# shizhenneko/Video-Transformer

Hardware: AMD Instinct MI355X
Metric: 720p frames/sec decoded+scored per node; segment-index exact-match vs CPU (higher is better)
Workload: dtype u8; 1 GPU; decode_score: BASELINE config [3] per-GPU share: 4 x 10-min 720p MP4 per GPU (config [3] = 32 videos over 8 GPUs; at N GPUs 4N videos, video i on rank i mod N) through vtseg.batch.plan_batch; synthetic H.264 1280x720 @30fps, 4 x 18000 frames (10.0 min) per GPU, thumbnails k=4; config_name=720p-batch, videos=4, videos_per_gpu=4, frames_per_video=18000, frames_per_gpu=72000, width=1280, height=720, k=4, parallelism=video-per-gpu x1 (video i on rank i mod 1), hw_queues=4, recon_launches=120, windows=1

## Files before the change

### video-transformer_amd/csrc/decode.hip

```cpp
#include <hip/hip_runtime.h>

#include <cstdint>

#include "common.h"
#include "decode.h"
#include "h264.h"
#include "parse_slice.h"
#include "pixel.h"

namespace vts {
namespace {

#ifndef VTS_PARSE_WAVES
#define VTS_PARSE_WAVES 0
#endif
#if VTS_PARSE_WAVES
#define VTS_PARSE_OCC __attribute__((amdgpu_waves_per_eu(VTS_PARSE_WAVES)))
#else
#define VTS_PARSE_OCC
#endif
__global__ void __launch_bounds__(64) VTS_PARSE_OCC h264_parse(ParseArgs a) {
  __shared__ ParseScratch scratch[64];
  const int s = blockIdx.x * blockDim.x + threadIdx.x;
  if (s >= a.n_slices) return;
  const SliceDesc sd = a.slices[s];
  const uint32_t errs = parse_slice(a.es, sd.nal_offset, sd.nal_size, sd.slot, sd.ref_slot, a.prm, a.cmd,
                                    &scratch[threadIdx.x], a.epoch);
  if (errs) atomicOr(a.err, errs);
}

__device__ __forceinline__ uint4 load16_any(const uint8_t *p) {
  const int sh = static_cast<int>(reinterpret_cast<uintptr_t>(p) & 15);
  const uint4 *q = reinterpret_cast<const uint4 *>(p - sh);
  const uint4 lo = q[0];
  if (sh == 0) return lo;
  const uint4 hi = q[1];
  const uint32_t w[8] = {lo.x, lo.y, lo.z, lo.w, hi.x, hi.y, hi.z, hi.w};
  const int qd = sh >> 2, r = sh & 3;
  uint32_t s[5];
#pragma unroll
  for (int i = 0; i < 5; ++i)
    s[i] = (qd == 0) ? w[i] : (qd == 1) ? w[i + 1] : (qd == 2) ? w[i + 2] : w[i + 3 < 8 ? i + 3 : 7];
  return make_uint4(__builtin_amdgcn_alignbyte(s[1], s[0], r), __builtin_amdgcn_alignbyte(s[2], s[1], r),
                    __builtin_amdgcn_alignbyte(s[3], s[2], r), __builtin_amdgcn_alignbyte(s[4], s[3], r));
}

__device__ __forceinline__ uint32_t has_zero_byte(uint32_t v) {
  return (v - 0x01010101u) & ~v & 0x80808080u;
}

__device__ bool epb_in_pcm(const uint8_t *chunk, int n, const uint8_t *pcm) {
  for (int j = -2; j < n; ++j) {
    const uint8_t *t = chunk + j;
    if (t + 2 < pcm || t + 2 >= pcm + 384) continue;
    if (t[0] == 0 && t[1] == 0 && t[2] == 3) return true;
  }
  return false;
}

__device__ __noinline__ uint32_t pcm_rows_epb(const uint8_t *pcm, int q, int kk, int hk) {
  bool bad = false;
  for (int i = 0; i < kk; ++i) bad |= epb_in_pcm(pcm + 16 * (q * kk + i), 16, pcm);
  for (int i = 0; i < hk; ++i)
    bad |= epb_in_pcm(pcm + 256 + 8 * (q * hk + i), 8, pcm) || epb_in_pcm(pcm + 320 + 8 * (q * hk + i), 8, pcm);
  return bad ? DEC_E_EPB_IN_PCM : 0u;
}

__device__ __forceinline__ uint4 interleave_uv(uint32_t u0, uint32_t u1, uint32_t v0, uint32_t v1) {
  return make_uint4(__builtin_amdgcn_perm(v0, u0, 0x05010400u), __builtin_amdgcn_perm(v0, u0, 0x07030602u),
                    __builtin_amdgcn_perm(v1, u1, 0x05010400u), __builtin_amdgcn_perm(v1, u1, 0x07030602u));
}

__device__ __forceinline__ int clampi(int v, int lo, int hi) { return v < lo ? lo : (v > hi ? hi : v); }

constexpr int kReconThreads = 256;

#ifndef VTS_NT_LOAD
#define VTS_NT_LOAD 0
#endif
#ifndef VTS_NT_STORE
#define VTS_NT_STORE 1
#endif
typedef uint32_t u32x4 __attribute__((ext_vector_type(4)));

__device__ __forceinline__ uint4 ld_row(const uint4 *p) {
#if VTS_NT_LOAD
  const u32x4 v = __builtin_nontemporal_load(reinterpret_cast<const u32x4 *>(p));
  return make_uint4(v.x, v.y, v.z, v.w);
#else
  return *p;
#endif
}
__device__ __forceinline__ void st_row(uint8_t *p, const uint4 v) {
#if VTS_NT_STORE
  __builtin_nontemporal_store(u32x4{v.x, v.y, v.z, v.w}, reinterpret_cast<u32x4 *>(p));
#else
  *reinterpret_cast<uint4 *>(p) = v;
#endif
}

struct FrameRefs {
  const uint8_t *es;
  const uint8_t *ref, *ref_uv;
  int W, H, CW, CH;
  int64_t pitch;
};

__device__ __forceinline__ uint4 fetch_row(const FrameRefs &F, uint64_t c, int r, int m, int mby,
                                           uint32_t &errs) {
  const uint32_t kind = static_cast<uint32_t>(c >> 62);
  const int mvx = static_cast<int16_t>(c & 0xffff), mvy = static_cast<int16_t>((c >> 16) & 0xffff);
  uint4 out = make_uint4(0, 0, 0, 0);
  if (kind == 0 || (kind == 2 && !F.ref)) {
    errs |= (kind == 0) ? DEC_E_MISSING_MB : DEC_E_NO_REF;
  } else if (r < 16) {
    if (kind == 1) {
      const uint8_t *pcm = F.es + static_cast<int64_t>(c & 0xffffffffffffull);
      const uint8_t *src = pcm + 16 * r;
      out = load16_any(src);
      if ((has_zero_byte(out.x) | has_zero_byte(out.y) | has_zero_byte(out.z) | has_zero_byte(out.w)) &&
          epb_in_pcm(src, 16, pcm))
        errs |= DEC_E_EPB_IN_PCM;
    } else {
      const int sy = clampi(mby * 16 + r + (mvy >> 2), 0, F.H - 1);
      const int sx = m * 16 + (mvx >> 2);
      const uint8_t *row = F.ref + sy * F.pitch;
      if (sx >= 0 && sx + 15 <= F.W - 1) {
        out = load16_any(row + sx);
      } else {
        uint64_t lo8 = 0, hi8 = 0;
#pragma unroll 1
        for (int b = 0; b < 16; ++b) {
          const uint64_t v = row[clampi(sx + b, 0, F.W - 1)];
          if (b < 8) lo8 |= v << (8 * b); else hi8 |= v << (8 * (b - 8));
        }
        out = make_uint4(uint32_t(lo8), uint32_t(lo8 >> 32), uint32_t(hi8), uint32_t(hi8 >> 32));
      }
    }
  } else {
    const int cr = r - 16;
    if (kind == 1) {
      const uint8_t *pcm = F.es + static_cast<int64_t>(c & 0xffffffffffffull);
      const uint4 u = load16_any(pcm + 256 + 8 * cr);
      const uint4 v = load16_any(pcm + 320 + 8 * cr);
      out = interleave_uv(u.x, u.y, v.x, v.y);
      if ((has_zero_byte(u.x) | has_zero_byte(u.y) | has_zero_byte(v.x) | has_zero_byte(v.y)) &&
          (epb_in_pcm(pcm + 256 + 8 * cr, 8, pcm) || epb_in_pcm(pcm + 320 + 8 * cr, 8, pcm)))
        errs |= DEC_E_EPB_IN_PCM;
    } else {
      const int fx = mvx & 7, fy = mvy & 7;
      const int cx = m * 8 + (mvx >> 3), cy = mby * 8 + cr + (mvy >> 3);
      if (fx == 0 && fy == 0) {
        const uint8_t *row = F.ref_uv + clampi(cy, 0, F.CH - 1) * F.pitch;
        if (cx >= 0 && cx + 7 <= F.CW - 1) {
          out = load16_any(row + 2 * cx);
        } else {
          uint64_t lo8 = 0, hi8 = 0;
#pragma unroll 1
          for (int b = 0; b < 8; ++b) {
            const int sx = clampi(cx + b, 0, F.CW - 1);
            const uint64_t v = uint64_t(row[2 * sx]) | (uint64_t(row[2 * sx + 1]) << 8);
            if (b < 4) lo8 |= v << (16 * b); else hi8 |= v << (16 * (b - 4));
          }
          out = make_uint4(uint32_t(lo8), uint32_t(lo8 >> 32), uint32_t(hi8), uint32_t(hi8 >> 32));
        }
      } else {
        const uint8_t *ra = F.ref_uv + clampi(cy, 0, F.CH - 1) * F.pitch;
        const uint8_t *rb = F.ref_uv + clampi(cy + 1, 0, F.CH - 1) * F.pitch;
        uint64_t lo8 = 0, hi8 = 0;
#pragma unroll 1
        for (int b = 0; b < 8; ++b) {
          const int xa = clampi(cx + b, 0, F.CW - 1), xb = clampi(cx + b + 1, 0, F.CW - 1);
          uint64_t pair = 0;
#pragma unroll
          for (int pl = 0; pl < 2; ++pl) {
            const int A = ra[2 * xa + pl], B = ra[2 * xb + pl], C = rb[2 * xa + pl], D = rb[2 * xb + pl];
            const uint64_t v = static_cast<uint64_t>(
                ((8 - fx) * (8 - fy) * A + fx * (8 - fy) * B + (8 - fx) * fy * C + fx * fy * D + 32) >> 6);
            pair |= v << (8 * pl);
          }
          if (b < 4) lo8 |= pair << (16 * b); else hi8 |= pair << (16 * (b - 4));
        }
        out = make_uint4(uint32_t(lo8), uint32_t(lo8 >> 32), uint32_t(hi8), uint32_t(hi8 >> 32));
      }
    }
  }
  return out;
}

__device__ __forceinline__ uint64_t current_cmd(uint64_t c, uint32_t epoch) {
  return ((c & kCmdEpochMask) >> kCmdEpochShift) == epoch ? (c & ~kCmdEpochMask) : 0;
}

__device__ __forceinline__ FrameRefs frame_refs(const ReconArgs &a, int ref_slot) {
  FrameRefs F;
  F.es = a.es;
  F.W = a.mb_width * 16;
  F.H = a.mb_height * 16;
  F.CW = F.W / 2;
  F.CH = F.H / 2;
  F.pitch = a.pitch;
  F.ref = ref_slot >= 0 ? a.surf + static_cast<int64_t>(ref_slot) * a.frame_stride : nullptr;
  F.ref_uv = F.ref ? F.ref + F.pitch * F.H : nullptr;
  return F;
}

__device__ __forceinline__ bool fast_cmd(const FrameRefs &F, uint64_t c) {
  const uint32_t kind = static_cast<uint32_t>(c >> 62);
  const int mvx = static_cast<int16_t>(c & 0xffff), mvy = static_cast<int16_t>((c >> 16) & 0xffff);
  return kind == 1 || (kind == 2 && F.ref && ((mvx | mvy) & 7) == 0);
}

__device__ __forceinline__ void issue_row(const FrameRefs &F, const uint8_t *pcmb, bool pcm, bool chroma,
                                          int rin, int m, int mby, int mvx, int mvy, uint4 &lo, uint4 &hi,
                                          int &shf) {
  if (pcm && chroma) {
    const uint8_t *pu = pcmb + 256 + 8 * rin;
    const int sh = static_cast<int>(reinterpret_cast<uintptr_t>(pu) & 7);
    const uint2 *au = reinterpret_cast<const uint2 *>(pu - sh);
    const uint2 u0 = au[0], u1 = au[1], v0 = au[8], v1 = au[9];
    shf = sh;
    lo = make_uint4(u0.x, u0.y, u1.x, u1.y);
    hi = make_uint4(v0.x, v0.y, v1.x, v1.y);
  } else {
    const uint4 *pa;
    int sh;
    if (pcm) {
      const uint8_t *p = pcmb + 16 * rin;
      sh = static_cast<int>(reinterpret_cast<uintptr_t>(p) & 15);
      pa = reinterpret_cast<const uint4 *>(p - sh);
    } else {
      const uint8_t *row = chroma ? F.ref_uv + clampi(mby * 8 + rin + (mvy >> 3), 0, F.CH - 1) * F.pitch
                                  : F.ref + clampi(mby * 16 + rin + (mvy >> 2), 0, F.H - 1) * F.pitch;
      const int x0 = chroma ? 2 * (m * 8 + (mvx >> 3)) : m * 16 + (mvx >> 2);
      if (x0 < 0) {
        pa = reinterpret_cast<const uint4 *>(row);
        sh = (x0 > -16 ? 16 + x0 : 0) | (1 << 8);
      } else if (x0 > F.W - 16) {
        pa = reinterpret_cast<const uint4 *>(row + F.W - 16);
        sh = min(x0 - (F.W - 16), 16) | (2 << 8);
      } else {
        const uint8_t *p = row + x0;
        sh = static_cast<int>(reinterpret_cast<uintptr_t>(p) & 15);
        pa = reinterpret_cast<const uint4 *>(p - sh);
      }
    }
    shf = sh;
    lo = ld_row(pa);
    hi = ld_row(sh >> 8 ? pa : pa + 1);
  }
}

__device__ __forceinline__ uint4 finish_row(bool chroma, bool pcm, uint4 lo, uint4 hi, int shf, uint32_t &zero) {
  if (pcm && chroma) {
    const int sh = shf & 7, qd = sh >> 2, r = sh & 3;
    const uint32_t a0 = qd ? lo.y : lo.x, a1 = qd ? lo.z : lo.y, a2 = qd ? lo.w : lo.z;
    const uint32_t b0 = qd ? hi.y : hi.x, b1 = qd ? hi.z : hi.y, b2 = qd ? hi.w : hi.z;
    const uint32_t ux = __builtin_amdgcn_alignbyte(a1, a0, r), uy = __builtin_amdgcn_alignbyte(a2, a1, r);
    const uint32_t vx = __builtin_amdgcn_alignbyte(b1, b0, r), vy = __builtin_amdgcn_alignbyte(b2, b1, r);
    zero |= has_zero_byte(ux) | has_zero_byte(uy) | has_zero_byte(vx) | has_zero_byte(vy);
    return interleave_uv(ux, uy, vx, vy);
  }
  if (!pcm && (shf >> 8)) {
    if ((shf >> 8) == 1) {
      const uint32_t f = chroma ? (hi.x & 0xffffu) * 0x00010001u : (hi.x & 0xffu) * 0x01010101u;
      lo = make_uint4(f, f, f, f);
    } else {
      const uint32_t g = chroma ? (lo.w >> 16) * 0x00010001u : (lo.w >> 24) * 0x01010101u;
      hi = make_uint4(g, g, g, g);
      if ((shf & 0xff) == 16) lo = hi;
    }
    shf &= 15;
  }
  const uint32_t w[8] = {lo.x, lo.y, lo.z, lo.w, hi.x, hi.y, hi.z, hi.w};
  const int qd = (shf >> 2) & 3, r = shf & 3;
  uint32_t t[5];
#pragma unroll
  for (int j = 0; j < 5; ++j)
    t[j] = (qd == 0) ? w[j] : (qd == 1) ? w[j + 1] : (qd == 2) ? w[j + 2] : w[j + 3 < 8 ? j + 3 : 7];
  const uint4 v = make_uint4(__builtin_amdgcn_alignbyte(t[1], t[0], r), __builtin_amdgcn_alignbyte(t[2], t[1], r),
                             __builtin_amdgcn_alignbyte(t[3], t[2], r), __builtin_amdgcn_alignbyte(t[4], t[3], r));
  if (pcm) zero |= has_zero_byte(v.x) | has_zero_byte(v.y) | has_zero_byte(v.z) | has_zero_byte(v.w);
  return v;
}

typedef uint4 uint4_a4 __attribute__((aligned(4)));
typedef uint32_t u32x3_a4 __attribute__((ext_vector_type(3), aligned(4)));
struct Row6 {
  uint32_t w0, w1, w2, w3, w4, w5;
  int shf;
};
__device__ __forceinline__ void issue_row6(const FrameRefs &F, const uint8_t *pcmb, bool pcm, bool chroma, int rin,
                                           int m, int mby, int mvx, int mvy, Row6 &o) {
  if (pcm && chroma) {
    const uint8_t *pu = pcmb + 256 + 8 * rin;
    const int sh = static_cast<int>(reinterpret_cast<uintptr_t>(pu) & 3);
    const u32x3_a4 a = *reinterpret_cast<const u32x3_a4 *>(pu - sh);
    const u32x3_a4 b = *reinterpret_cast<const u32x3_a4 *>(pu + 64 - sh);
    o.w0 = a.x, o.w1 = a.y, o.w2 = a.z, o.w3 = b.x, o.w4 = b.y, o.w5 = b.z;
    o.shf = sh | (3 << 8);
    return;
  }
  const uint8_t *p;
  int mode = 0, esh = 0;
  if (pcm) {
    p = pcmb + 16 * rin;
  } else {
    const uint8_t *row = chroma ? F.ref_uv + clampi(mby * 8 + rin + (mvy >> 3), 0, F.CH - 1) * F.pitch
                                : F.ref + clampi(mby * 16 + rin + (mvy >> 2), 0, F.H - 1) * F.pitch;
    const int x0 = chroma ? 2 * (m * 8 + (mvx >> 3)) : m * 16 + (mvx >> 2);
    if (x0 < 0) {
      p = row;
      mode = 1;
      esh = x0 > -16 ? 16 + x0 : 0;
    } else if (x0 > F.W - 16) {
      p = row + F.W - 16;
      mode = 2;
// ... 996 lines not shown
```

### video-transformer_amd/csrc/parse_slice.h

```cpp
#pragma once
#include <cstdint>

#include "h264.h"

#if defined(__HIPCC__)
#define VTS_HD __host__ __device__
#else
#define VTS_HD
#endif
#define VTS_INLINE inline __attribute__((always_inline))
#define VTS_UNLIKELY(x) __builtin_expect(!!(x), 0)

namespace vts {

VTS_HD VTS_INLINE uint32_t vts_alignbyte(uint32_t hi, uint32_t lo, int r) {
  return static_cast<uint32_t>(((static_cast<uint64_t>(hi) << 32) | lo) >> (8 * (r & 3)));
}
VTS_HD VTS_INLINE int vts_min(int a, int b) { return a < b ? a : b; }
VTS_HD VTS_INLINE int vts_max(int a, int b) { return a > b ? a : b; }

struct alignas(16) Cmd2 {
  uint64_t a, b;
};

template <int kW>
struct WinBitsT {
  const uint8_t *base;
  int64_t abs0;
  uint64_t win;
  int32_t nb;
  int32_t fill;
  int32_t real;
  int32_t size;
  int32_t pos;
  int32_t zeros;
  int32_t epb;
  int32_t epb_next;
  int32_t cache_at;
  uint32_t *cache;
  bool err;

  VTS_HD VTS_INLINE void init(const uint8_t *p, int64_t abs, int32_t n, uint32_t *scratch) {
    cache = scratch;
    base = p;
    abs0 = abs;
    size = n;
    win = 0;
    nb = fill = real = pos = zeros = epb = 0;
    epb_next = -1;
    cache_at = -1;
    err = false;
  }
  VTS_HD VTS_INLINE uint32_t load4(int32_t i) {
    constexpr int32_t kBlk = 4 * (kW - 1);
    const int32_t blk = i - (i % kBlk);
    if (blk != cache_at) {
      const uint8_t *pb = base + blk;
      const int sh = static_cast<int>(reinterpret_cast<uintptr_t>(pb) & 3);
      uint32_t t[kW + 1];
      if constexpr (kW > 5) {
        const uint32_t *w = reinterpret_cast<const uint32_t *>(reinterpret_cast<uintptr_t>(pb) & ~uintptr_t(3));
#pragma unroll
        for (int k = 0; k <= kW; ++k) t[k] = w[k];
      } else {
        const uint32_t *w = reinterpret_cast<const uint32_t *>(pb - sh);
#pragma unroll
        for (int k = 0; k <= kW; ++k) t[k] = w[k];
      }
#pragma unroll
      for (int k = 0; k < kW; ++k) cache[k] = sh ? vts_alignbyte(t[k + 1], t[k], sh) : t[k];
      cache_at = blk;
    }
    const int32_t o = i - blk, q = o >> 2, r = o & 3;
    return vts_alignbyte(cache[q + 1], cache[q], r);
  }
  VTS_HD VTS_INLINE void refill() {
    const uint32_t v = load4(pos);
    const uint32_t x = v ^ 0x03030303u;
    if (pos + 4 <= size && !((x - 0x01010101u) & ~x & 0x80808080u)) {
      win |= static_cast<uint64_t>(__builtin_bswap32(v)) << (32 - nb);
      nb += 32;
      fill += 32;
      real += 32;
      pos += 4;
      zeros = (v >> 24) ? 0 : (((v >> 16) & 0xffu) ? 1 : 2);
      return;
    }
#pragma unroll 1
    for (int i = 0; i < 4; ++i) {
      if (pos >= size) {
        nb += 8;
        fill += 8;
        continue;
      }
      const uint32_t b = (v >> (8 * i)) & 0xffu;
      ++pos;
      if (zeros >= 2 && b == 3) {
        ++epb;
        zeros = 0;
        epb_next = real >> 3;
        continue;
      }
      zeros = b ? 0 : vts_min(zeros + 1, 2);
      win |= static_cast<uint64_t>(b) << (56 - nb);
      nb += 8;
      fill += 8;
      real += 8;
    }
  }
  VTS_HD VTS_INLINE void ensure(int n) {
    while (nb < n) refill();
  }
  VTS_HD VTS_INLINE void skip(int n) {
    win <<= n;
    nb -= n;
  }
  VTS_HD VTS_INLINE uint32_t bits(int n) {
    if (n == 0) return 0;
    ensure(n);
    const uint32_t v = static_cast<uint32_t>(win >> (64 - n));
    skip(n);
    return v;
  }
  VTS_HD VTS_INLINE uint32_t bit() { return bits(1); }
  VTS_HD VTS_INLINE uint32_t ue() {
    ensure(32);
    const uint32_t p = static_cast<uint32_t>(win >> 32);
    if (p == 0) {
      err = true;
      return 0;
    }
    const int lz = __builtin_clz(p);
    if (lz < 16) {
      const int len = 2 * lz + 1;
      skip(len);
      return (p >> (32 - len)) - 1u;
    }
    skip(lz + 1);
    return ((1u << lz) - 1u) + bits(lz);
  }
  VTS_HD VTS_INLINE int32_t se() {
    const uint32_t k = ue();
    return (k & 1u) ? static_cast<int32_t>((k + 1) >> 1) : -static_cast<int32_t>(k >> 1);
  }
  VTS_HD VTS_INLINE int32_t consumed() const { return fill - nb; }
  VTS_HD VTS_INLINE void align() { skip(nb & 7); }
  VTS_HD VTS_INLINE bool overrun() const { return consumed() > real; }
  VTS_HD VTS_INLINE bool more(int32_t stop_byte, int64_t stop_bit) const {
    if (pos < stop_byte) return true;
    return consumed() < stop_bit - 8ll * epb;
  }
  VTS_HD VTS_INLINE int64_t skip_raw(int32_t n, bool &epb_hit) {
    const int32_t r = consumed() >> 3;
    epb_hit = epb_next >= r;
    const int32_t e = r + epb;
    const int64_t off = abs0 + e;
    reset_at(e + n, (r + n) * 8);
    return off;
  }
  VTS_HD VTS_INLINE void reset_at(int32_t e, int32_t rb) {
    pos = e;
    if (pos > size) err = true;
    win = 0;
    nb = 0;
    fill = real = rb;
    const uint32_t w = load4(vts_max(pos - 2, 0));
    const uint32_t b2 = w & 0xffu, b1 = (w >> 8) & 0xffu;
    zeros = (b1 != 0) ? 0 : ((b2 != 0) ? 1 : 2);
  }
};
using WinBits = WinBitsT<5>;

VTS_HD VTS_INLINE int median3(int a, int b, int c) {
  return vts_max(vts_min(a, b), vts_min(vts_max(a, b), c));
}

struct Nb {
  bool avail;
  int ref;
  int mvx, mvy;
};

VTS_HD VTS_INLINE Nb nb_from_cmd(uint64_t c) {
  Nb n{true, -1, 0, 0};
  if ((c >> 62) == 2) {
    n.ref = 0;
    n.mvx = static_cast<int16_t>(c & 0xffff);
    n.mvy = static_cast<int16_t>((c >> 16) & 0xffff);
  }
  return n;
}

struct CmdWriter {
  uint64_t *cmd;
  Cmd2 *e;
  int64_t gbase;
  uint64_t tag;
  int32_t g;
  uint32_t mask;

  VTS_HD VTS_INLINE void init(uint64_t *c, int64_t gb, Cmd2 *scratch, uint64_t epoch_tag) {
    cmd = c;
    e = scratch;
    tag = epoch_tag;
    gbase = gb;
    g = -1;
    mask = 0;
  }
  VTS_HD VTS_INLINE void flush() {
    if (!mask) return;
    uint64_t *p = cmd + g;
    if (mask == 0xfu) {
      Cmd2 *q = reinterpret_cast<Cmd2 *>(p);
      q[0] = e[0];
      q[1] = e[1];
    } else {
      const uint64_t *el = reinterpret_cast<const uint64_t *>(e);
      if (mask & 1u) p[0] = el[0];
      if (mask & 2u) p[1] = el[1];
      if (mask & 4u) p[2] = el[2];
      if (mask & 8u) p[3] = el[3];
    }
    mask = 0;
  }
  VTS_HD VTS_INLINE void put(int32_t addr, uint64_t c) {
    const int32_t j = static_cast<int32_t>((gbase + addr) & 3);
    const int32_t ga = addr - j;
    if (ga != g) {
      flush();
      g = ga;
    }
    reinterpret_cast<uint64_t *>(e)[j] = c | tag;
    mask |= 1u << j;
    if (j == 3) flush();
  }
  VTS_HD VTS_INLINE uint64_t get(int32_t addr) const {
    const uint64_t in_group = reinterpret_cast<const uint64_t *>(e)[(addr - g) & 3];
    const uint64_t in_memory = cmd[addr];
    return (mask && addr >= g && addr < g + 4) ? in_group : in_memory;
  }
};

struct ParseScratch {
  Cmd2 cmd[2];
  uint32_t cache[6];
};

VTS_HD VTS_INLINE uint32_t parse_slice(const uint8_t *es, int64_t nal_offset, int32_t nal_size, int32_t slot,
                                       int32_t ref_slot, const H264DevParams &P, uint64_t *cmd_all,
                                       ParseScratch *scratch, uint32_t epoch = 0) {
  const int nmb = P.mb_width * P.mb_height;
  CmdWriter out;
  out.init(cmd_all + static_cast<int64_t>(slot) * nmb, static_cast<int64_t>(slot) * nmb, scratch->cmd,
           static_cast<uint64_t>(epoch) << kCmdEpochShift);
  uint32_t errs = 0;

  const uint8_t *nal = es + nal_offset;
  const uint32_t hdr = nal[0];
  const int nal_type = hdr & 0x1f, nal_ref_idc = (hdr >> 5) & 3;
  WinBits br;
  br.init(nal + 1, nal_offset + 1, nal_size - 1, scratch->cache);
  int32_t last = nal_size - 1;
  while (last > 0 && nal[last] == 0) --last;
  if (last <= 0) return DEC_E_SYNTAX;
  const uint32_t lb = nal[last];
  const int tz = __builtin_ctz(lb);
  const int32_t stop_byte = last - 1;
  const int64_t stop_bit = int64_t(stop_byte) * 8 + (7 - tz);

  const int first_mb = static_cast<int>(br.ue());
  int slice_type = static_cast<int>(br.ue());
  if (slice_type > 4) slice_type -= 5;
  const int pps_id = static_cast<int>(br.ue());
  if (pps_id != P.pps_id) errs |= DEC_E_PPS;
  br.bits(P.log2_max_frame_num);
  if (nal_type == 5) br.ue();
  if (P.poc_type == 0) {
    br.bits(P.log2_max_poc_lsb);
    if (P.bottom_field_pic_order_in_frame_present) br.se();
  } else if (P.poc_type == 1 && !P.delta_pic_order_always_zero) {
    br.se();
    if (P.bottom_field_pic_order_in_frame_present) br.se();
  }
  if (P.redundant_pic_cnt_present) {
    if (br.ue() != 0) errs |= DEC_E_SYNTAX;
  }
  const bool is_p = (slice_type == 0);
  if (!is_p && slice_type != 2) errs |= DEC_E_SLICE_TYPE;
  int num_ref = P.num_ref_idx_l0_default_active;
  if (is_p) {
    if (br.bit()) num_ref = static_cast<int>(br.ue()) + 1;
    if (br.bit()) errs |= DEC_E_REFLIST;
    if (num_ref != 1) errs |= DEC_E_MULTIREF;
    if (ref_slot < 0) errs |= DEC_E_NO_REF;
  }
  if (nal_ref_idc != 0) {
    if (nal_type == 5) {
      br.bit();
      br.bit();
    } else if (br.bit()) {
      errs |= DEC_E_MMCO;
    }
  }
  const int qp = P.pic_init_qp + br.se();
  int deblock_idc = 0, alpha_off = 0;
  if (P.deblocking_filter_control_present) {
    deblock_idc = static_cast<int>(br.ue());
    if (deblock_idc != 1) {
      alpha_off = 2 * br.se();
      br.se();
    }
  }
  const int cqp_up = P.chroma_qp_index_offset > 0 ? P.chroma_qp_index_offset : 0;
  if (deblock_idc != 1 && qp + cqp_up + alpha_off >= 16) errs |= DEC_E_DEBLOCK;
  if (first_mb < 0 || first_mb >= nmb) errs |= DEC_E_SYNTAX;
  if (errs || br.err || br.overrun()) return errs | ((br.err || br.overrun()) ? DEC_E_SYNTAX : 0u);

  int addr = first_mb;
  const int mbw = P.mb_width;
  int x = addr % mbw, y = addr / mbw;
  Nb left{false, -1, 0, 0};
  bool more = true;
  bool fresh = false;
  while (more && addr < nmb) {
    if (is_p) {
      const int skip = static_cast<int>(br.ue());
      if (br.err || addr + skip > nmb) {
        errs |= DEC_E_SYNTAX;
        break;
      }
      for (int i = 0; i < skip; ++i) {
        const bool a_ok = x > 0 && addr - 1 >= first_mb;
        const bool b_ok = y > 0 && addr - mbw >= first_mb;
        int mvx = 0, mvy = 0;
        if (a_ok && b_ok) {
          const Nb A = left;
          const Nb B = nb_from_cmd(out.get(addr - mbw));
          if (!(A.ref == 0 && A.mvx == 0 && A.mvy == 0) && !(B.ref == 0 && B.mvx == 0 && B.mvy == 0)) {
            const bool c_ok = x < mbw - 1 && addr - mbw + 1 >= first_mb;
            const bool d_ok = x > 0 && addr - mbw - 1 >= first_mb;
            const Nb C = c_ok ? nb_from_cmd(out.get(addr - mbw + 1))
                              : (d_ok ? nb_from_cmd(out.get(addr - mbw - 1)) : Nb{false, -1, 0, 0});
            const int match = (A.ref == 0) + (B.ref == 0) + (C.ref == 0);
            if (match == 1) {
              mvx = (A.ref == 0) ? A.mvx : (B.ref == 0) ? B.mvx : C.mvx;
              mvy = (A.ref == 0) ? A.mvy : (B.ref == 0) ? B.mvy : C.mvy;
            } else {
              mvx = median3(A.mvx, B.mvx, C.mvx);
              mvy = median3(A.mvy, B.mvy, C.mvy);
            }
          }
        }
        if ((mvx & 3) || (mvy & 3)) errs |= DEC_E_SUBPEL;
        out.put(addr, MB_INTER | (uint64_t(uint16_t(mvx))) | (uint64_t(uint16_t(mvy)) << 16));
        left = Nb{true, 0, mvx, mvy};
        ++addr;
        if (++x == mbw) {
          x = 0;
          ++y;
        }
      }
      if (skip > 0) {
        more = br.more(stop_byte, stop_bit);
        fresh = false;
      }
      if (!more || addr >= nmb) break;
    }
    if (!is_p && fresh) {
      uint32_t hit = 0;
#pragma unroll
      for (int j = 0; j < 8; ++j) {
        const int64_t q = static_cast<int64_t>(br.pos) + 386 * j;
        if ((q + 386) * 8 <= stop_bit && addr + j < nmb && nal[1 + q] == 0x0D && nal[2 + q] == 0x00)
          hit |= 1u << j;
      }
      const int ok = __builtin_ctz(~hit);
      if (ok > 0 && br.zeros < 2) {
        for (int j = 0; j < ok; ++j)
          out.put(addr + j, MB_PCM | static_cast<uint64_t>(br.abs0 + br.pos + 386 * j + 2));
        addr += ok;
        x += ok;
        while (x >= mbw) {
          x -= mbw;
          ++y;
        }
        left = Nb{true, -1, 0, 0};
        br.reset_at(br.pos + 386 * ok, br.consumed() + 386 * 8 * ok);
        more = br.more(stop_byte, stop_bit);
        continue;
      }
    }
    fresh = false;
    const int mb_type = static_cast<int>(br.ue());
    if ((!is_p && mb_type == 25) || (is_p && mb_type == 30)) {
      br.align();
      bool hit = false;
      const int64_t off = br.skip_raw(384, hit);
      if (hit) errs |= DEC_E_EPB_IN_PCM;
      out.put(addr, MB_PCM | static_cast<uint64_t>(off));
      left = Nb{true, -1, 0, 0};
      fresh = true;
    } else if (is_p && mb_type == 0) {
      const int mvdx = br.se(), mvdy = br.se();
      const uint32_t cbp_code = br.ue();
      if (cbp_code != 0) errs |= DEC_E_RESIDUAL;
      const bool a_ok = x > 0 && addr - 1 >= first_mb;
      const bool b_ok = y > 0 && addr - mbw >= first_mb;
      const bool c_ok = y > 0 && x < mbw - 1 && addr - mbw + 1 >= first_mb;
      const bool d_ok = y > 0 && x > 0 && addr - mbw - 1 >= first_mb;
      Nb A = a_ok ? left : Nb{false, -1, 0, 0};
      Nb B = b_ok ? nb_from_cmd(out.get(addr - mbw)) : Nb{false, -1, 0, 0};
      Nb C = c_ok ? nb_from_cmd(out.get(addr - mbw + 1))
                  : (d_ok ? nb_from_cmd(out.get(addr - mbw - 1)) : Nb{false, -1, 0, 0});
      if (!B.avail && !C.avail && A.avail) B = C = A;
      int px, py;
      const int match = (A.ref == 0) + (B.ref == 0) + (C.ref == 0);
      if (match == 1) {
        px = (A.ref == 0) ? A.mvx : (B.ref == 0) ? B.mvx : C.mvx;
        py = (A.ref == 0) ? A.mvy : (B.ref == 0) ? B.mvy : C.mvy;
      } else {
        px = median3(A.mvx, B.mvx, C.mvx);
        py = median3(A.mvy, B.mvy, C.mvy);
      }
      const int mvx = px + mvdx, mvy = py + mvdy;
      if ((mvx & 3) || (mvy & 3)) errs |= DEC_E_SUBPEL;
      if (mvx < -32768 || mvx > 32767 || mvy < -32768 || mvy > 32767) errs |= DEC_E_SYNTAX;
      out.put(addr, MB_INTER | (uint64_t(uint16_t(mvx))) | (uint64_t(uint16_t(mvy)) << 16));
      left = Nb{true, 0, mvx, mvy};
    } else {
      errs |= DEC_E_MB_TYPE;
      break;
    }
    ++addr;
    if (++x == mbw) {
      x = 0;
      ++y;
    }
    if (br.err || br.overrun()) break;
    more = br.more(stop_byte, stop_bit);
  }
  out.flush();
  if (br.err || br.overrun()) errs |= DEC_E_SYNTAX;
  return errs;
}

}
```

Baseline: 1.692 million frames/s.

## Batch runs of skipped and zero-mvd P macroblocks in slice parser

```diff
diff --git a/video-transformer_amd/csrc/decode.hip b/video-transformer_amd/csrc/decode.hip
--- a/video-transformer_amd/csrc/decode.hip
+++ b/video-transformer_amd/csrc/decode.hip
@@ -12,7 +12,7 @@
 namespace {
 
 #ifndef VTS_PARSE_WAVES
-#define VTS_PARSE_WAVES 0
+#define VTS_PARSE_WAVES (VTS_PARSE_RUNS ? 6 : 0)
 #endif
 #if VTS_PARSE_WAVES
 #define VTS_PARSE_OCC __attribute__((amdgpu_waves_per_eu(VTS_PARSE_WAVES)))
diff --git a/video-transformer_amd/csrc/parse_slice.h b/video-transformer_amd/csrc/parse_slice.h
--- a/video-transformer_amd/csrc/parse_slice.h
+++ b/video-transformer_amd/csrc/parse_slice.h
@@ -10,6 +10,9 @@
 #endif
 #define VTS_INLINE inline __attribute__((always_inline))
 #define VTS_UNLIKELY(x) __builtin_expect(!!(x), 0)
+#ifndef VTS_PARSE_RUNS
+#define VTS_PARSE_RUNS 1
+#endif
 
 namespace vts {
 
@@ -234,6 +237,41 @@
     mask |= 1u << j;
     if (j == 3) flush();
   }
+  VTS_HD VTS_INLINE void put_slots(int32_t ga, uint32_t m, uint64_t c) {
+    if (ga != g) {
+      flush();
+      g = ga;
+    }
+    uint64_t *el = reinterpret_cast<uint64_t *>(e);
+    if (m & 1u) el[0] = c;
+    if (m & 2u) el[1] = c;
+    if (m & 4u) el[2] = c;
+    if (m & 8u) el[3] = c;
+    mask |= m;
+    if (m & 8u) flush();
+  }
+  VTS_HD VTS_INLINE void put_run(int32_t addr, int32_t n, uint64_t c) {
+    c |= tag;
+    const int32_t j = static_cast<int32_t>((gbase + addr) & 3);
+    if (j) {
+      const int32_t h = vts_min(4 - j, n);
+      put_slots(addr - j, ((1u << h) - 1u) << j, c);
+      addr += h;
+      n -= h;
+    }
+    if (n >= 4) {
+      flush();
+      const Cmd2 v{c, c};
+      do {
+        Cmd2 *q = reinterpret_cast<Cmd2 *>(cmd + addr);
+        q[0] = v;
+        q[1] = v;
+        addr += 4;
+        n -= 4;
+      } while (n >= 4);
+    }
+    if (n > 0) put_slots(addr, (1u << n) - 1u, c);
+  }
   VTS_HD VTS_INLINE uint64_t get(int32_t addr) const {
     const uint64_t in_group = reinterpret_cast<const uint64_t *>(e)[(addr - g) & 3];
     const uint64_t in_memory = cmd[addr];
@@ -261,9 +299,31 @@
   WinBits br;
   br.init(nal + 1, nal_offset + 1, nal_size - 1, scratch->cache);
   int32_t last = nal_size - 1;
+#if VTS_PARSE_RUNS
+  uint32_t lb = 0;
+  while (last >= 4) {
+    const uint8_t *p = nal + last - 3;
+    const int sh = static_cast<int>(reinterpret_cast<uintptr_t>(p) & 3);
+    const uint32_t *w = reinterpret_cast<const uint32_t *>(p - sh);
+    const uint32_t v = sh ? vts_alignbyte(w[1], w[0], sh) : w[0];
+    if (v) {
+      const int zb = __builtin_clz(v) >> 3;
+      last -= zb;
+      lb = (v >> (8 * (3 - zb))) & 0xffu;
+      break;
+    }
+    last -= 4;
+  }
+  if (!lb) {
+    while (last > 0 && nal[last] == 0) --last;
+    if (last <= 0) return DEC_E_SYNTAX;
+    lb = nal[last];
+  }
+#else
   while (last > 0 && nal[last] == 0) --last;
   if (last <= 0) return DEC_E_SYNTAX;
   const uint32_t lb = nal[last];
+#endif
   const int tz = __builtin_ctz(lb);
   const int32_t stop_byte = last - 1;
   const int64_t stop_bit = int64_t(stop_byte) * 8 + (7 - tz);
@@ -322,6 +382,158 @@
   Nb left{false, -1, 0, 0};
   bool more = true;
   bool fresh = false;
+#if VTS_PARSE_RUNS
+  constexpr int kRunChunk = 8;
+  int pend = 0;
+  bool got_run = false;
+  const int top_c = x != 0;
+  while (pend > 0 || (more && addr < nmb)) {
+    const bool in_skip = pend > 0;
+    int n = 0;
+    if (is_p) {
+      if (in_skip) {
+        n = vts_min(pend, kRunChunk);
+      } else if (!got_run) {
+        br.ensure(32);
+        const uint64_t inv = ~br.win;
+        int ones = inv ? __builtin_clzll(inv) : 64;
+        if (br.pos >= stop_byte) {
+          const int64_t room = stop_bit - 8ll * br.epb - br.consumed();
+          if (room < ones) ones = room < 0 ? 0 : static_cast<int>(room);
+        }
+        n = ones / 5;
+      }
+      n = vts_min(n, mbw - x);
+    }
+    const int n_top = first_mb + mbw - addr - (in_skip ? 0 : top_c);
+    if (n > 0 && n_top > 0) {
+      n = vts_min(n, n_top);
+      int mvx = 0, mvy = 0;
+      if (!in_skip && x > 0 && addr - 1 >= first_mb) {
+        mvx = left.mvx;
+        mvy = left.mvy;
+      }
+      if ((mvx & 3) || (mvy & 3)) errs |= DEC_E_SUBPEL;
+      out.put_run(addr, n, MB_INTER | (uint64_t(uint16_t(mvx))) | (uint64_t(uint16_t(mvy)) << 16));
+      left = Nb{true, 0, mvx, mvy};
+      addr += n;
+      x += n;
+      if (x == mbw) {
+        x = 0;
+        ++y;
+      }
+      if (in_skip) {
+        pend -= n;
+        if (pend == 0) more = br.more(stop_byte, stop_bit);
+      } else {
+        br.skip(5 * n);
+        more = br.more(stop_byte, stop_bit);
+      }
+      continue;
+    }
+    int mvdx = 0, mvdy = 0;
+    bool inter = n > 0;
+    if (inter) {
+      if (!in_skip) br.skip(5);
+    } else {
+      if (is_p && !got_run) {
+        const int skip = static_cast<int>(br.ue());
+        if (br.err || addr + skip > nmb) {
+          errs |= DEC_E_SYNTAX;
+          break;
+        }
+        if (skip > 0) {
+          pend = skip;
+          got_run = true;
+          continue;
+        }
+      }
+      got_run = false;
+      if (!is_p && fresh) {
+        uint32_t hit = 0;
+#pragma unroll
+        for (int j = 0; j < 8; ++j) {
+          const int64_t q = static_cast<int64_t>(br.pos) + 386 * j;
+          if ((q + 386) * 8 <= stop_bit && addr + j < nmb && nal[1 + q] == 0x0D && nal[2 + q] == 0x00)
+            hit |= 1u << j;
+        }
+        const int ok = __builtin_ctz(~hit);
+        if (ok > 0 && br.zeros < 2) {
+          for (int j = 0; j < ok; ++j)
+            out.put(addr + j, MB_PCM | static_cast<uint64_t>(br.abs0 + br.pos + 386 * j + 2));
+          addr += ok;
+          x += ok;
+          while (x >= mbw) {
+            x -= mbw;
+            ++y;
+          }
+          left = Nb{true, -1, 0, 0};
+          br.reset_at(br.pos + 386 * ok, br.consumed() + 386 * 8 * ok);
+          more = br.more(stop_byte, stop_bit);
+          continue;
+        }
+      }
+      fresh = false;
+      const int mb_type = static_cast<int>(br.ue());
+      if ((!is_p && mb_type == 25) || (is_p && mb_type == 30)) {
+        br.align();
+        bool hit = false;
+        const int64_t off = br.skip_raw(384, hit);
+        if (hit) errs |= DEC_E_EPB_IN_PCM;
+        out.put(addr, MB_PCM | static_cast<uint64_t>(off));
+        left = Nb{true, -1, 0, 0};
+        fresh = true;
+      } else if (is_p && mb_type == 0) {
+        mvdx = br.se();
+        mvdy = br.se();
+        if (br.ue() != 0) errs |= DEC_E_RESIDUAL;
+        inter = true;
+      } else {
+        errs |= DEC_E_MB_TYPE;
+        break;
+      }
+    }
+    if (inter) {
+      const bool a_ok = x > 0 && addr - 1 >= first_mb;
+      const bool b_ok = y > 0 && addr - mbw >= first_mb;
+      const bool c_ok = y > 0 && x < mbw - 1 && addr - mbw + 1 >= first_mb;
+      const bool d_ok = y > 0 && x > 0 && addr - mbw - 1 >= first_mb;
+      Nb A = a_ok ? left : Nb{false, -1, 0, 0};
+      Nb B = b_ok ? nb_from_cmd(out.get(addr - mbw)) : Nb{false, -1, 0, 0};
+      Nb C = c_ok ? nb_from_cmd(out.get(addr - mbw + 1))
+                  : (d_ok ? nb_from_cmd(out.get(addr - mbw - 1)) : Nb{false, -1, 0, 0});
+      const bool still = !(a_ok && b_ok) || (A.ref == 0 && A.mvx == 0 && A.mvy == 0) ||
+                         (B.ref == 0 && B.mvx == 0 && B.mvy == 0);
+      if (!B.avail && !C.avail && A.avail) B = C = A;
+      int px, py;
+      const int match = (A.ref == 0) + (B.ref == 0) + (C.ref == 0);
+      if (match == 1) {
+        px = (A.ref == 0) ? A.mvx : (B.ref == 0) ? B.mvx : C.mvx;
+        py = (A.ref == 0) ? A.mvy : (B.ref == 0) ? B.mvy : C.mvy;
+      } else {
+        px = median3(A.mvx, B.mvx, C.mvx);
+        py = median3(A.mvy, B.mvy, C.mvy);
+      }
+      int mvx = px + mvdx, mvy = py + mvdy;
+      if (in_skip && still) mvx = mvy = 0;
+      if ((mvx & 3) || (mvy & 3)) errs |= DEC_E_SUBPEL;
+      if (mvx < -32768 || mvx > 32767 || mvy < -32768 || mvy > 32767) errs |= DEC_E_SYNTAX;
+      out.put(addr, MB_INTER | (uint64_t(uint16_t(mvx))) | (uint64_t(uint16_t(mvy)) << 16));
+      left = Nb{true, 0, mvx, mvy};
+    }
+    ++addr;
+    if (++x == mbw) {
+      x = 0;
+      ++y;
+    }
+    if (in_skip) {
+      if (--pend == 0) more = br.more(stop_byte, stop_bit);
+    } else {
+      if (br.err || br.overrun()) break;
+      more = br.more(stop_byte, stop_bit);
+    }
+  }
+#else
   while (more && addr < nmb) {
     if (is_p) {
       const int skip = static_cast<int>(br.ue());
@@ -439,6 +651,7 @@
     if (br.err || br.overrun()) break;
     more = br.more(stop_byte, stop_bit);
   }
+#endif
   out.flush();
   if (br.err || br.overrun()) errs |= DEC_E_SYNTAX;
   return errs;
```

New measurement: 1.696 million frames/s, median of 2. About the same (+0.3%).
